# jrobine/actor-critic

Measured on AMD Instinct MI355X. Metric: env-steps/sec (whole node) + ACKTR update ms, Breakout 84x84x4, higher is better.
Workload: dtype fp32

## Files before the change

actor-critic_amd/actorcritic/_lib.py:

```python

import ctypes
import os

import torch

_HERE = os.path.dirname(os.path.abspath(__file__))
LIB_PATH = os.path.join(os.path.dirname(_HERE), 'libacmi.so')
if os.environ.get('ACMI_LIB'):
    LIB_PATH = os.environ['ACMI_LIB']

c_int = ctypes.c_int
c_i64 = ctypes.c_int64
c_u32 = ctypes.c_uint32
c_float = ctypes.c_float
c_vp = ctypes.c_void_p


class AcmiError(RuntimeError):
    """A libacmi entry point returned a non-zero status."""


class Net(ctypes.Structure):
    _fields_ = [('num_actions', c_int), ('conv3_filters', c_int), ('params', c_vp), ('conv_prep', c_vp),
                ('gemm_mode', c_int), ('forward_mode', c_int), ('conv_stats_mode', c_int)]


class Acts(ctypes.Structure):
    _fields_ = [('a1', c_vp), ('a2', c_vp), ('a3', c_vp), ('a4', c_vp),
                ('logits', c_vp), ('value', c_vp), ('ld_logits', c_int),
                ('ws', c_vp), ('ws_floats', c_i64), ('m1', c_vp), ('m2', c_vp), ('m3', c_vp)]


class Bwd(ctypes.Structure):
    _fields_ = [('d1', c_vp), ('d2', c_vp), ('d3', c_vp), ('d4', c_vp),
                ('dhead', c_vp), ('ldh', c_int)]


class EnvState(ctypes.Structure):
    _fields_ = [('episode', c_vp), ('step', c_vp), ('length', c_vp), ('total', c_vp), ('done', c_vp),
                ('game', c_vp)]


class RolloutIO(ctypes.Structure):
    _fields_ = [('seed', c_u32), ('stream_id', c_u32), ('counter', c_u32), ('counter_dev', c_vp),
                ('row_offset', c_int), ('actions', c_vp), ('bad_rows', c_vp), ('state', EnvState),
                ('env_offset', c_int), ('env_seed', c_u32), ('obs_out', c_vp), ('out_stride', c_i64),
                ('rewards', c_vp), ('terminals', c_vp), ('episode_rewards', c_vp), ('ld', c_i64),
                ('tower_done', c_int), ('next_acts', c_vp), ('next_act_stride', c_i64), ('obs_copy', c_vp)]


_SIGS = {
    'acmi_last_error': (ctypes.c_char_p, []),
    'acmi_abi_version': (c_int, []),
    'acmi_abi_struct_sizes': (c_int, [c_vp, c_int]),
    'acmi_set_forward_mode': (c_int, [c_int]),
    'acmi_get_forward_mode': (c_int, []),
    'acmi_set_gemm_mode': (c_int, [c_int]),
    'acmi_get_gemm_mode': (c_int, []),
    'acmi_set_conv_stats_mode': (c_int, [c_int]),
    'acmi_get_conv_stats_mode': (c_int, []),
    'acmi_band_info': (c_int, [c_int, c_int, c_i64, ctypes.POINTER(c_i64)]),
    'acmi_param_count': (c_i64, [c_int, c_int]),
    'acmi_conv_prep_bytes': (c_i64, [c_int]),
    'acmi_kfac_packed_floats': (c_i64, [c_int, c_int, c_int]),
    'acmi_kfac_pack': (c_int, [c_int, c_int, c_int, c_vp, c_vp, c_vp]),
    'acmi_kfac_unpack': (c_int, [c_int, c_int, c_int, c_vp, c_vp, c_vp]),
    'acmi_conv_prepare': (c_int, [ctypes.POINTER(Net), c_vp, c_vp]),
    'acmi_param_offsets': (c_int, [c_int, c_int, ctypes.POINTER(c_i64)]),
    'acmi_kfac_layout': (c_int, [c_int, c_int, ctypes.POINTER(c_i64), ctypes.POINTER(c_i64),
                                 ctypes.POINTER(c_i64), ctypes.POINTER(c_i64)]),
    'acmi_forward': (c_int, [ctypes.POINTER(Net), c_vp, c_i64, c_int, ctypes.POINTER(Acts), c_int, c_vp]),
    'acmi_forward_ws_floats': (c_i64, [c_int]),
    'acmi_forward_strided': (c_int, [ctypes.POINTER(Net), c_vp, c_i64, c_int, ctypes.POINTER(Acts), c_int,
                                     c_i64, c_vp]),
    'acmi_sample_actions': (c_int, [c_vp, c_int, c_int, c_int, c_u32, c_u32, c_u32, c_vp, c_int, c_vp,
                                    c_vp, c_vp]),
    'acmi_sample_actions_at': (c_int, [c_vp, c_int, c_int, c_int, c_u32, c_u32, c_u32, c_int, c_vp, c_int,
                                       c_vp, c_vp, c_vp]),
    'acmi_sample_actions_dev': (c_int, [c_vp, c_int, c_int, c_int, c_u32, c_u32, c_vp, c_u32, c_int, c_vp,
                                        c_int, c_vp, c_vp, c_vp]),
    'acmi_rollout_step': (c_int, [ctypes.POINTER(Net), c_vp, c_i64, c_int, ctypes.POINTER(Acts), c_i64,
                                  ctypes.POINTER(RolloutIO), c_vp]),
    'acmi_categorical': (c_int, [c_vp, c_int, c_int, c_int, c_vp, c_vp, c_vp, c_vp]),
    'acmi_returns': (c_int, [c_vp, c_vp, c_vp, c_vp, c_int, c_int, c_vp, c_vp, c_vp, c_vp, c_vp]),
    'acmi_gae': (c_int, [c_vp, c_vp, c_vp, c_vp, c_int, c_int, c_float, c_float, c_vp, c_vp, c_vp]),
    'acmi_adv_moments_ws_doubles': (c_i64, [c_i64]),
    'acmi_adv_moments': (c_int, [c_vp, c_i64, c_vp, c_vp, c_vp]),
    'acmi_adv_normalize': (c_int, [c_vp, c_i64, c_vp, ctypes.c_double, ctypes.c_double, c_vp]),
    'acmi_a2c_loss_ws_floats': (c_i64, [c_int]),
    'acmi_a2c_loss': (c_int, [c_vp, c_int, c_vp, c_vp, c_vp, c_vp, c_int, c_int, c_float, c_float, c_float,
                              c_vp, c_int, c_vp, c_vp, c_vp]),
    'acmi_ppo_loss_ws_floats': (c_i64, [c_int]),
    'acmi_ppo_loss': (c_int, [c_vp, c_int, c_vp, c_vp, c_vp, c_vp, c_vp, c_vp, c_int, c_int, c_float, c_float,
                              c_float, c_float, c_float, c_vp, c_int, c_vp, c_vp, c_vp, c_vp]),
    'acmi_backward_ws_floats': (c_i64, [c_int, c_int, c_int]),
    'acmi_backward': (c_int, [ctypes.POINTER(Net), c_vp, c_i64, c_int, ctypes.POINTER(Acts),
                              ctypes.POINTER(Bwd), c_vp, c_vp, c_vp, c_i64, c_vp]),
    'acmi_kfac_output_stats': (c_int, [ctypes.POINTER(Net), c_int, ctypes.POINTER(Acts), ctypes.POINTER(Bwd),
                                       c_u32, c_u32, c_u32, c_vp, c_vp, c_i64, c_vp]),
    'acmi_backward_stacked': (c_int, [ctypes.POINTER(Net), c_vp, c_i64, c_int, ctypes.POINTER(Acts),
                                      ctypes.POINTER(Bwd), c_vp, c_vp, c_vp, c_i64, ctypes.POINTER(Bwd), c_u32, c_u32,
                                      c_u32, c_vp, c_i64, c_vp]),
    'acmi_kfac_output_stats_finish': (c_int, [ctypes.POINTER(Net), c_int, ctypes.POINTER(Acts), ctypes.POINTER(Bwd),
                                              c_vp, c_vp, c_i64, c_vp]),
    'acmi_debug_ws_flushes': (c_int, []),
    'acmi_debug_convt2': (c_int, [ctypes.POINTER(Net), c_int, c_vp, c_vp, c_vp, c_vp, c_int, c_vp, c_vp, c_vp, c_vp,
                                  c_vp]),
    'acmi_kfac_ema': (c_int, [c_vp, c_vp, c_vp, c_i64, c_float, c_float, c_float, c_vp]),
    'acmi_kfac_inverse_layout': (c_int, [c_int, c_int, ctypes.POINTER(c_i64), ctypes.POINTER(c_i64)]),
    'acmi_kfac_inverse_floats': (c_i64, [c_int, c_int]),
    'acmi_kfac_inverse_ws_doubles': (c_i64, [c_int, c_int]),
    'acmi_kfac_inverse': (c_int, [c_int, c_int, c_vp, c_float, c_int, c_vp, c_vp, c_vp]),
    'acmi_kfac_eig_ws_doubles': (c_i64, [c_int, c_int]),
    'acmi_kfac_eigvals': (c_int, [c_int, c_int, c_vp, c_vp, c_vp, c_vp]),
    'acmi_kfac_step_ws_floats': (c_i64, [c_int, c_int]),
    'acmi_kfac_step': (c_int, [c_int, c_int, c_vp, c_vp, c_vp, c_vp, c_float, c_float, c_float, c_vp, c_vp,
                               c_vp, c_vp]),
    'acmi_opt_ws_floats': (c_i64, [c_i64]),
    'acmi_momentum_apply': (c_int, [c_vp, c_vp, c_vp, c_i64, c_float, c_float, c_float, c_vp, c_vp, c_vp]),
    'acmi_rmsprop_apply': (c_int, [c_vp, c_vp, c_vp, c_vp, c_i64, c_float, c_float, c_float, c_float, c_float,
                                   c_vp, c_vp, c_vp]),
    'acmi_adam_apply': (c_int, [c_vp, c_vp, c_vp, c_vp, c_i64, c_float, c_float, c_float, c_float, c_float,
                                c_vp, c_vp, c_vp]),
    'acmi_env_reset': (c_int, [ctypes.POINTER(EnvState), c_int, c_int, c_u32, c_vp, c_i64, c_vp]),
    'acmi_env_step': (c_int, [ctypes.POINTER(EnvState), c_int, c_int, c_u32, c_vp, c_vp, c_i64, c_vp, c_i64,
                              c_vp, c_vp, c_vp, c_i64, c_vp]),
    'acmi_atari_preprocess': (c_int, [c_vp, c_i64, c_i64, c_vp, c_int, c_int, c_int, c_vp, c_i64, c_vp]),
    'acmi_atari_stack': (c_int, [c_vp, c_i64, c_i64, c_vp, c_int, c_int, c_int, c_vp, c_int, c_vp, c_vp,
                                 c_i64, c_vp]),
    'acmi_stream_wait_backward_dx': (c_int, [c_vp]),
    'acmi_selftest_plans': (c_int, [c_int]),
    'acmi_gemm_f32': (c_int, [c_vp, c_vp, c_vp, c_int, c_int, c_int, c_vp]),
    'acmi_prof_enable': (c_int, [c_int, c_int]),
    'acmi_prof_collect': (c_int, [ctypes.POINTER(ctypes.c_double), ctypes.POINTER(c_int)]),
}

GEMM_F32 = 0
GEMM_X3 = 1
FWD_F32 = 0
FWD_BF16 = 1

CONV_STATS_PATCHES = 0
CONV_STATS_BAND = 1

PROF_CONV1_WGRAD = 1
PROF_CONV2_WGRAD = 2
PROF_CONV1_FWD = 3
PROF_CONV1_AFACTOR = 4
PROF_CONV2_DX = 5

EXPORTED = tuple(_SIGS)

_lib = None


def load():
    global _lib
    if _lib is None:
        if not os.path.exists(LIB_PATH):
            raise ImportError('libacmi.so not found at {} - build it with `python __graft_entry__.py build` '
                              '(hipcc --offload-arch=gfx950); there is no CPU fallback'.format(LIB_PATH))
        lib = ctypes.CDLL(LIB_PATH)
        for name, (res, args) in _SIGS.items():
            if os.environ.get('ACMI_LIB') and not hasattr(lib, name):
                continue
            fn = getattr(lib, name)
            fn.restype = res
            fn.argtypes = args
        if lib.acmi_abi_version() != 4:
            raise ImportError('libacmi ABI mismatch')
        _lib = lib
    return _lib


def check(status, what=''):
    if status != 0:
        msg = load().acmi_last_error().decode(errors='replace')
        raise AcmiError('{} failed ({}): {}'.format(what, status, msg))


def call(name, *args):
    check(getattr(load(), name)(*args), name)


def ptr(t):
    if t is None:
        return None
    assert t.is_contiguous(), 'libacmi needs contiguous buffers'
    return ctypes.c_void_p(t.data_ptr())

# ... 10 lines not shown
```

actor-critic_amd/csrc/convt2.hpp:

```cpp
#pragma once

#include "f16x2.hpp"
#include "gemm.hpp"

namespace acmi {

struct CT2 {
  static constexpr int CIN = 32, COUT = 64, OH = 9, OW = 9, PW = 10, L = 100;
  static constexpr int NKS = 16;
  static constexpr int STEP_BYTES = 4 * 2 * 1024;
  static constexpr int FRAG_BYTES = NKS * STEP_BYTES;
  static constexpr int BYTES = FRAG_BYTES + 4 * kAmaxWords;
  static constexpr int TILE = 128;
};

__device__ __forceinline__ void convt2_wmax_body(const float* w2, char* out, int b, int nb) {
  float m = 0.f;
  for (int i = b * 256 + threadIdx.x; i < 16 * CT2::CIN * CT2::COUT; i += nb * 256)
    m = fmaxf(m, fabsf(w2[i]));
  m = wave_max(m);
  if ((threadIdx.x & 63) == 0) amax_update(reinterpret_cast<unsigned*>(out + CT2::FRAG_BYTES), m);
}

__device__ __forceinline__ void convt2_prep_body(const float* w2, char* out, int blk) {
// ... 176 lines not shown
#pragma unroll
        for (int q = 0; q < 4; ++q) {
          float4 o;
          if constexpr (MASK) {
            o.x = (bits[q] & 1u) ? v[q].x : 0.f;
            o.y = (bits[q] & 2u) ? v[q].y : 0.f;
            o.z = (bits[q] & 4u) ? v[q].z : 0.f;
            o.w = (bits[q] & 8u) ? v[q].w : 0.f;
          } else {
            o.x = xa[q].x > 0.f ? v[q].x : 0.f;
            o.y = xa[q].y > 0.f ? v[q].y : 0.f;
            o.z = xa[q].z > 0.f ? v[q].z : 0.f;
            o.w = xa[q].w > 0.f ? v[q].w : 0.f;
          }
          if (jok[q]) {
            *reinterpret_cast<float4*>(d1 + (long long)(pix[q] + dp) * CT2::CIN + ri) = o;
            d1am = absmax4(d1am, o);
          }
        }
        __builtin_amdgcn_fence(__ATOMIC_RELEASE, "wavefront");
        __builtin_amdgcn_wave_barrier();
        __builtin_amdgcn_fence(__ATOMIC_ACQUIRE, "wavefront");
      }
    } else {
#pragma unroll
      for (int p = 0; p < 4; ++p) {
        const int py = p >> 1, px = p & 1;
        const long long pix = ((long long)n * 20 + 2 * Y + py) * 20 + 2 * X + px;
#pragma unroll
        for (int g = 0; g < 4; ++g) {
          const int ci = 8 * g + 4 * hl;
          float4 x;
          if constexpr (MASK) {
            const uint32_t b = *reinterpret_cast<const uint32_t*>(jok ? a1 + pix : zero) >> ci;
            x = make_float4((float)(b & 1u), (float)((b >> 1) & 1u), (float)((b >> 2) & 1u), (float)((b >> 3) & 1u));
          } else {
            x = *reinterpret_cast<const float4*>(jok ? a1 + pix * CT2::CIN + ci : zero);
          }
          const int c = lane & 31;
          scr[(ci + 0) * 36 + c] = x.x > 0.f ? acc[p][4 * g + 0] : 0.f;
          scr[(ci + 1) * 36 + c] = x.y > 0.f ? acc[p][4 * g + 1] : 0.f;
          scr[(ci + 2) * 36 + c] = x.z > 0.f ? acc[p][4 * g + 2] : 0.f;
          scr[(ci + 3) * 36 + c] = x.w > 0.f ? acc[p][4 * g + 3] : 0.f;
        }
        __builtin_amdgcn_wave_barrier();
#pragma unroll
        for (int h = 0; h < 2; ++h) {
          const float* rp = scr + (lane & 31) * 36 + 16 * h + 8 * hl;
          const float4 x0 = *reinterpret_cast<const float4*>(rp);
          const float4 x1 = *reinterpret_cast<const float4*>(rp + 4);
          uint4 hh, mm, ll;
          split3(x0.x, x0.y, hh.x, mm.x, ll.x);
          split3(x0.z, x0.w, hh.y, mm.y, ll.y);
          split3(x1.x, x1.y, hh.z, mm.z, ll.z);
          split3(x1.z, x1.w, hh.w, mm.w, ll.w);
          const bf16x8 f[3] = {__builtin_bit_cast(bf16x8, hh), __builtin_bit_cast(bf16x8, mm),
                               __builtin_bit_cast(bf16x8, ll)};
          gacc = mfma_x3(f, f, gacc);
        }
        __builtin_amdgcn_wave_barrier();
      }
    }
    __syncthreads();
  }

  if constexpr (MIX || !GRAM) amax_publish(d1max, d1am, lane);
  if constexpr (MIX || GRAM) {
    float* red = reinterpret_cast<float*>(lds);
    for (int w = 0; w < 4; ++w) {
      if (wave == w) {
#pragma unroll
        for (int r = 0; r < 16; ++r) {
          const int i = (r & 3) + 8 * (r >> 2) + 4 * hl, jc = lane & 31;
          red[i * 32 + jc] = (w ? red[i * 32 + jc] : 0.f) + gacc[r];
        }
      }
      __syncthreads();
    }
    float* out = gpart + (long long)blockIdx.x * 33 * 32;
    for (int e = tid; e < 32 * 32; e += 256) out[e] = red[e];
  }
}

#ifndef ACMI_CT2_STORE_BLOCKS
#define ACMI_CT2_STORE_BLOCKS 0
#endif
inline int convt2_store_blocks(int B) {
  const int ntiles = (B * CT2::L + CT2::TILE - 1) / CT2::TILE;
  return ACMI_CT2_STORE_BLOCKS > 0 ? std::max(1, std::min(ntiles, ACMI_CT2_STORE_BLOCKS)) : ntiles;
}
inline int convt2_gram_blocks(int B) {
  const int ntiles = (B * CT2::L + CT2::TILE - 1) / CT2::TILE;
  return std::max(1, std::min(ntiles, 768));
}

}
```

actor-critic_amd/csrc/net.hip:

```cpp
#include <math.h>
#include <stdlib.h>
#include <stdarg.h>
#include <stdio.h>
#include <string.h>

#include <vector>

#include "gemm.hpp"
#include "gemm3.hpp"
#include "conv1u8.hpp"
#include "convt3.hpp"
#include "convfwd3.hpp"
#include "band.hpp"
#include "tower.hpp"
#include "fc4roll.hpp"
#include "convt2.hpp"
#include "stepper.hpp"
#include "towersplit.hpp"

namespace acmi {

static int s_gemm_mode = [] {
  const char* e = getenv("ACMI_GEMM");
  return (e && e[0] == 'f') ? ACMI_GEMM_F32 : ACMI_GEMM_X3;
}();
static int s_conv_stats_mode = [] {
  const char* e = getenv("ACMI_BAND");
  return (e && e[0] == '0') ? ACMI_CONV_STATS_PATCHES : ACMI_CONV_STATS_BAND;
}();
static int s_forward_mode = [] {
  const char* e = getenv("ACMI_FORWARD");
  return (e && e[0] == 'b') ? ACMI_FWD_BF16 : ACMI_FWD_F32;
}();
thread_local int g_gemm_mode = s_gemm_mode;
thread_local int g_conv_stats_mode = s_conv_stats_mode;
thread_local int g_forward_mode = s_forward_mode;

static bool net_modes_ok(const acmi_net_t* n) {
  if (!n) return true;
  const int g = n->gemm_mode ? n->gemm_mode - 1 : s_gemm_mode;
  const int f = n->forward_mode ? n->forward_mode - 1 : s_forward_mode;
  const int c = n->conv_stats_mode ? n->conv_stats_mode - 1 : s_conv_stats_mode;
  return (g == ACMI_GEMM_F32 || g == ACMI_GEMM_X3) && (f == ACMI_FWD_F32 || f == ACMI_FWD_BF16) &&
         (c == ACMI_CONV_STATS_PATCHES || c == ACMI_CONV_STATS_BAND) && (f == ACMI_FWD_F32 || g == ACMI_GEMM_X3);
}
struct ModeScope {
  int g, f, c;
  explicit ModeScope(const acmi_net_t* n) : g(g_gemm_mode), f(g_forward_mode), c(g_conv_stats_mode) {
    g_gemm_mode = n && n->gemm_mode ? n->gemm_mode - 1 : s_gemm_mode;
    g_forward_mode = n && n->forward_mode ? n->forward_mode - 1 : s_forward_mode;
    g_conv_stats_mode = n && n->conv_stats_mode ? n->conv_stats_mode - 1 : s_conv_stats_mode;
  }
  ~ModeScope() {
    g_gemm_mode = g;
    g_forward_mode = f;
    g_conv_stats_mode = c;
  }
};

static thread_local char g_err[512];
void set_error(const char* fmt, ...) {
  va_list ap;
  va_start(ap, fmt);
  vsnprintf(g_err, sizeof(g_err), fmt, ap);
  va_end(ap);
}

static int g_prof_site = 0;
static int g_prof_cap = 0;
static int g_prof_n = 0;
static hipEvent_t* g_prof_ev = nullptr;

static void prof_begin(int site, hipStream_t s) {
  if (site != g_prof_site || g_prof_n >= g_prof_cap) return;
  (void)hipEventRecord(g_prof_ev[2 * g_prof_n], s);
}
static void prof_end(int site, hipStream_t s) {
  if (site != g_prof_site || g_prof_n >= g_prof_cap) return;
  (void)hipEventRecord(g_prof_ev[2 * g_prof_n + 1], s);
  ++g_prof_n;
}

struct Layout {
  int A, C3;
  long long off[12];
  long long total;
  long long K[6], N[6];
  long long din[6], dout[6];
// ... 1114 lines not shown
    }
    m = std::max(m, gcov_plan(co[l], rowsL[l]).floats);
  }
  m = std::max(m, band_ws_floats(band_host_plan(20, 20, 32, 4, 4, 2, 64), B));
  m = std::max(m, band_ws_floats(band_host_plan(9, 9, 64, 3, 3, 1, C3), B));
  return (m + 63) / 64 * 64;
}

static long long afactor_ws_floats(int B) { return conv1_afactor_ws_ints(400LL * B); }

static long long head_grad_ldg(int A) { return roundup4(A + 1) < 8 ? 8 : roundup4(A + 1); }
static long long bwd_prefix_floats(int B) { return kBandScratch + (afactor_ws_floats(B) + 63) / 64 * 64; }
static long long stats_prefix_floats(int B, int A) { return kBandScratch + ((long long)B * head_grad_ldg(A) + 63) / 64 * 64; }
static int g_ws_flushes = 0;

static hipEvent_t* dx_done_event() {
  static hipEvent_t ev[64] = {};
  int dev = 0;
  if (hipGetDevice(&dev) != hipSuccess || dev < 0 || dev >= 64) return nullptr;
  if (!ev[dev] && hipEventCreateWithFlags(&ev[dev], hipEventDisableTiming) != hipSuccess) {
    ev[dev] = nullptr;
    return nullptr;
  }
  return &ev[dev];
}
template <int C3>
static int dx_chain_pre(const Layout& L, const float* P, int B, const acmi_acts_t* a,
                        const acmi_bwd_t* bw, const float* dhead, int ldh,
                        hipStream_t s, const char* prep, unsigned* dxs) {
  ACMI_REQUIRE(dxs, ACMI_ERR_ARG, "dx_chain: no scratch");
  ACMI_REQUIRE(hipMemsetAsync(dxs, 0, kBandScratch * sizeof(unsigned), s) == hipSuccess, ACMI_ERR_HIP,
               "dx_chain: scratch reset failed");
  if (L.A == 4 && ldh % 4 == 0 && (uintptr_t)(P + L.off[8]) % 16 == 0 && (uintptr_t)dhead % 16 == 0)
    hipLaunchKernelGGL(heads_dx4_kernel, dim3(cdiv((long long)B * 128, 256)), dim3(256), 0, s, dhead,
                       ldh, B, P + L.off[8], P + L.off[10], a->a4, bw->d4, dxs + kBsMaxD4);
  else
    hipLaunchKernelGGL(heads_dx_kernel, dim3(cdiv((long long)B * 128, 256)), dim3(256), 0, s, dhead,
                       ldh, B, P + L.off[8], P + L.off[10], L.A, a->a4, bw->d4, dxs + kBsMaxD4);
  const unsigned* hdr = prep ? reinterpret_cast<const unsigned*>(prep + TowerPrep<C3>::HDR) : nullptr;
  const unsigned* w3max = hdr ? hdr + kTowMaxW3 : dxs + kBsMaxW3;
  const unsigned* w4max = hdr ? hdr + kTowMaxW4 : dxs + kBsMaxW4;
  if (!hdr && g_gemm_mode == ACMI_GEMM_X3) {
    hipLaunchKernelGGL(absmax_kernel, dim3(16), dim3(256), 0, s, P + L.off[4], (long long)576 * C3,
                       dxs + kBsMaxW3);
    hipLaunchKernelGGL(absmax_kernel, dim3(64), dim3(256), 0, s, P + L.off[6], (long long)49 * C3 * 512,
                       dxs + kBsMaxW4);
  }
  {
    const int K3 = 49 * C3;
    RowsAsK<DenseRows> opA{DenseRows{bw->d4, 512, B, 512}};
    MatTK<true> opB{P + L.off[6], 512, 512, K3};
    auto run = [&](auto epi) {
      if (g_gemm_mode == ACMI_GEMM_X3)
        launch_gemm3_f16<128, 64, 32, 2, 1>(opA, opB, epi, B, K3, 512, dxs + kBsMaxD4, w4max, s);
      else
        launch_mm<64, 128, 32, 1, 2, false, false, 16>(opA, opB, epi, B, K3, 512, 1, 0, s);
    };
    prof_begin(ACMI_PROF_FC4_DX, s);
    if (a->m3) run(EpiReluGrad<true>{bw->d3, reinterpret_cast<const float*>(a->m3), K3, dxs + kBsMaxD3});
    else run(EpiReluGrad<false>{bw->d3, a->a3, K3, dxs + kBsMaxD3});
    prof_end(ACMI_PROF_FC4_DX, s);
  }
  {
    const char* ct3p = prep ? prep + TowerPrep<C3>::BYTES + CT2::BYTES + fc4_prep_bytes(49 * C3) : nullptr;
    using Src = ConvTRows<9, 9, 3, 3, 1, C3>;
    using W = ConvTWeights<3, 3, 1, 64, C3>;
    W opA{P + L.off[4]};
    RowsAsK<Src> opB{Src{bw->d3, B * Src::L}};
    auto run = [&](auto epi) {
      if (g_gemm_mode == ACMI_GEMM_X3)
        launch_convt_x3<9, 9, 3, 3, 1, 64, C3, 256>(P + L.off[4], ct3p, bw->d3, B, epi, w3max, dxs + kBsMaxD3, s);
      else
        launch_mm<64, 128, 16, 1, 2, false, false, 16>(opA, opB, epi, W::N, B * Src::L, Src::COLS, 1, 0, s);
    };
    prof_begin(ACMI_PROF_CONV3_DX, s);
    if (a->m2) run(EpiConvT<9, 9, 1, 64, true>{bw->d2, reinterpret_cast<const float*>(a->m2), dxs + kBsMaxD2});
    else run(EpiConvT<9, 9, 1, 64>{bw->d2, a->a2, dxs + kBsMaxD2});
    prof_end(ACMI_PROF_CONV3_DX, s);
  }
  ACMI_LAUNCH_CHECK("dx_chain");
  return ACMI_OK;
}

template <int C3>
static int dx_conv2(const Layout& L, const float* P, int B, const acmi_acts_t* a, const acmi_bwd_t* bw,
                    hipStream_t s, const char* prep, float* gram_part, bool* gram_done, unsigned* dxs) {
  if (gram_done) *gram_done = false;
  {
    using Src = ConvTRows<20, 20, 4, 4, 2, 64>;
    using W = ConvTWeights<4, 4, 2, 32, 64>;
    W opA{P + L.off[2]};
    RowsAsK<Src> opB{Src{bw->d2, B * Src::L}};
    const float* act1 = a->m1 ? reinterpret_cast<const float*>(a->m1) : a->a1;
    prof_begin(ACMI_PROF_CONV2_DX, s);
    const char* p2 = prep ? prep + TowerPrep<C3>::BYTES : nullptr;
    if (p2 && g_gemm_mode == ACMI_GEMM_X3) {
      auto go = [&](auto GRAMc, auto MASKc) {
        constexpr bool GR = decltype(GRAMc)::value, MK = decltype(MASKc)::value;
        if (GR)
          hipLaunchKernelGGL((convt2_kernel<GR, MK>), dim3(convt2_gram_blocks(B)), dim3(256), 0, s, p2, bw->d2,
                             act1, nullptr, B, gram_part, dxs + kBsMaxD2, nullptr);
        else
          hipLaunchKernelGGL((convt2_kernel<GR, MK>), dim3(convt2_store_blocks(B)), dim3(256), 0, s, p2,
                             bw->d2, act1, bw->d1, B, nullptr, dxs + kBsMaxD2, dxs + kBsMaxD1);
      };
      using T = std::true_type;
      using F = std::false_type;
      if (gram_part) {
        if (a->m1) go(T{}, T{});
        else go(T{}, F{});
        if (gram_done) *gram_done = true;
      } else {
        if (a->m1) go(F{}, T{});
        else go(F{}, F{});
      }
    } else if (a->m1) {
      launch_mm<128, 128, 16, 2, 2, false, false, 16>(
          opA, opB, EpiConvT<20, 20, 2, 32, true>{bw->d1, act1, dxs + kBsMaxD1}, W::N, B * Src::L, Src::COLS, 1, 0, s);
    } else {
      launch_mm<128, 128, 16, 2, 2, false, false, 16>(opA, opB, EpiConvT<20, 20, 2, 32>{bw->d1, act1, dxs + kBsMaxD1},
                                                      W::N, B * Src::L, Src::COLS, 1, 0, s);
    }
    prof_end(ACMI_PROF_CONV2_DX, s);
  }
  ACMI_LAUNCH_CHECK("dx_conv2");
  return ACMI_OK;
}

template <int C3>
static int dx_chain(const Layout& L, const float* P, int B, const acmi_acts_t* a,
                    const acmi_bwd_t* bw, const float* dhead, int ldh,
                    hipStream_t s, const char* prep = nullptr, float* gram_part = nullptr,
                    bool* gram_done = nullptr, unsigned* dxs = nullptr) {
  const int rc = dx_chain_pre<C3>(L, P, B, a, bw, dhead, ldh, s, prep, dxs);
  if (rc) return rc;
  return dx_conv2<C3>(L, P, B, a, bw, s, prep, gram_part, gram_done, dxs);
}

template <int C3>
static int backward_impl(const Layout& L, const float* P, const uint8_t* obs,
                         long long img_stride, int B, const acmi_acts_t* a,
                         const acmi_bwd_t* bw, float* grads, float* astat,
                         float* ws, long long ws_cap, hipStream_t s, const char* prep,
                         bool dx_done = false) {
  const bool st = astat != nullptr;
  const bool fuse_c1 = st && g_gemm_mode == ACMI_GEMM_X3;
  unsigned* bscr = reinterpret_cast<unsigned*>(ws);
  const long long prefix = bwd_prefix_floats(B);
  float* part = ws + prefix;
  const long long avail = ws_cap - prefix;
  const bool band = band_on(st);
  int rc = ACMI_OK;
  if (!dx_done) {
    rc = dx_chain<C3>(L, P, B, a, bw, bw->dhead, bw->ldh, s, prep, nullptr, nullptr, bscr);
    if (rc) return rc;
    hipEvent_t* ev = dx_done_event();
    ACMI_REQUIRE(ev && hipEventRecord(*ev, s) == hipSuccess, ACMI_ERR_HIP, "acmi_backward: dX event record failed");
  }
  float* wpart_c1 = nullptr;
  if (st) {
    prof_begin(ACMI_PROF_CONV1_AFACTOR, s);
    const int rc0 = conv1_afactor_u8(obs, img_stride, B, astat + L.stat_off[0],
                                     reinterpret_cast<int*>(ws + kBandScratch), afactor_ws_floats(B), s,
                                     fuse_c1 ? bw->d1 : nullptr, &wpart_c1, bscr + kBsMaxD1);
    prof_end(ACMI_PROF_CONV1_AFACTOR, s);
    if (rc0) return rc0;
  }
  WgradSet fin;
  long long off = 0;
  auto flush = [&]() {
    if (fin.n) hipLaunchKernelGGL(finalize_wgrad_multi_kernel, dim3(fin.blocks), dim3(256), 0, s, fin);
    fin = WgradSet();
    off = 0;
  };
  if (st && fuse_c1) {
    const long long rows = 400LL * B;
    WgradDesc d{wpart_c1, conv1_afactor_fused_chunks(rows), 256, 32, 0, 32, grads + L.off[0], 32,
                nullptr, nullptr, (int)rows, 1.0f / 255.0f};
    fin.add(d, 0, 0, fin_blocks(d));
  }
  auto layer = [&](long long need, auto&& run) -> int {
    long long used = 0;
// ... 509 lines not shown
  const char* prep = static_cast<const char*>(net->conv_prep);
  if (L.C3 == 32)
    return output_stats_impl<32>(L, net->params, B, acts, bwd_s, 0, 0, 0, g_stats, ws_s, ws_s_floats, s, prep, 2);
  return output_stats_impl<64>(L, net->params, B, acts, bwd_s, 0, 0, 0, g_stats, ws_s, ws_s_floats, s, prep, 2);
}

int acmi_stream_wait_backward_dx(acmi_stream_t stream) {
  hipEvent_t* ev = dx_done_event();
  ACMI_REQUIRE(ev && hipStreamWaitEvent((hipStream_t)stream, *ev, 0) == hipSuccess, ACMI_ERR_HIP,
               "acmi_stream_wait_backward_dx failed");
  return ACMI_OK;
}

int acmi_kfac_output_stats(const acmi_net_t* net, int B, const acmi_acts_t* acts,
                           const acmi_bwd_t* bwd, uint32_t seed, uint32_t row_offset,
                           uint32_t counter, float* g_stats, float* ws, int64_t ws_floats,
                           acmi_stream_t stream) {
  ACMI_REQUIRE(net_modes_ok(net), ACMI_ERR_ARG, "acmi_kfac_output_stats: bad acmi_net_t mode fields");
  const ModeScope mode_scope(net);
  Layout L;
  ACMI_REQUIRE(net && acts && bwd && g_stats && ws, ACMI_ERR_ARG,
               "acmi_kfac_output_stats: null argument");
  ACMI_REQUIRE(make_layout(net->num_actions, net->conv3_filters, &L), ACMI_ERR_ARG, "bad net");
  ACMI_REQUIRE(B > 0 && spans32(B, 400 * 32, 400 * 32), ACMI_ERR_ARG, "bad B");
  ACMI_REQUIRE(masks_ok(acts), ACMI_ERR_ARG, "acmi_kfac_output_stats: ReLU masks m1..m3 must be all set or all NULL");
  const long long need = acmi_backward_ws_floats(B, net->num_actions, net->conv3_filters);
  ACMI_REQUIRE(ws_floats >= need, ACMI_ERR_WS, "acmi_kfac_output_stats: workspace of %lld floats < %lld",
               (long long)ws_floats, need);
  hipStream_t s = (hipStream_t)stream;
  if (L.C3 == 32)
    return output_stats_impl<32>(L, net->params, B, acts, bwd, seed, row_offset, counter,
                                 g_stats, ws, ws_floats, s, static_cast<const char*>(net->conv_prep));
  return output_stats_impl<64>(L, net->params, B, acts, bwd, seed, row_offset, counter, g_stats,
                               ws, ws_floats, s, static_cast<const char*>(net->conv_prep));
}

int acmi_prof_enable(int site, int capacity) {
  ACMI_REQUIRE(site >= 0 && capacity >= 0 && capacity <= 65536, ACMI_ERR_ARG,
               "acmi_prof_enable: bad site/capacity");
  if (g_prof_ev) {
    for (int i = 0; i < 2 * g_prof_cap; ++i) (void)hipEventDestroy(g_prof_ev[i]);
    delete[] g_prof_ev;
    g_prof_ev = nullptr;
  }
  g_prof_site = 0;
  g_prof_cap = 0;
  g_prof_n = 0;
  if (site == 0 || capacity == 0) return ACMI_OK;
  g_prof_ev = new hipEvent_t[2 * capacity];
  for (int i = 0; i < 2 * capacity; ++i) {
    if (hipEventCreate(&g_prof_ev[i]) != hipSuccess) {
      set_error("acmi_prof_enable: hipEventCreate failed");
      return ACMI_ERR_HIP;
    }
  }
  g_prof_site = site;
  g_prof_cap = capacity;
  return ACMI_OK;
}

int acmi_prof_collect(double* total_ms, int* count) {
  ACMI_REQUIRE(total_ms && count, ACMI_ERR_ARG, "acmi_prof_collect: null argument");
  double t = 0.0;
  for (int i = 0; i < g_prof_n; ++i) {
    if (hipEventSynchronize(g_prof_ev[2 * i + 1]) != hipSuccess) {
      set_error("acmi_prof_collect: hipEventSynchronize failed");
      return ACMI_ERR_HIP;
    }
    float ms = 0.f;
    (void)hipEventElapsedTime(&ms, g_prof_ev[2 * i], g_prof_ev[2 * i + 1]);
    t += ms;
  }
  *total_ms = t;
  *count = g_prof_n;
  g_prof_n = 0;
  return ACMI_OK;
}

int acmi_debug_convt2(const acmi_net_t* net, int mode, const float* d2a, const float* d2b, const uint32_t* m1,
                      float* d1, int B, float* gram_part, const uint32_t* d2max_a, const uint32_t* d2max_b,
                      uint32_t* d1max, acmi_stream_t stream) {
  ACMI_REQUIRE(net_modes_ok(net), ACMI_ERR_ARG, "acmi_debug_convt2: bad acmi_net_t mode fields");
  const ModeScope mode_scope(net);
  ACMI_REQUIRE(net && net->conv_prep && d2a && d2b && m1 && d1 && gram_part && d2max_a && d2max_b && d1max && B > 0,
               ACMI_ERR_ARG, "acmi_debug_convt2: bad arguments");
  const char* p2 = static_cast<const char*>(net->conv_prep) +
                   (net->conv3_filters == 32 ? TowerPrep<32>::BYTES : TowerPrep<64>::BYTES);
  hipStream_t s = (hipStream_t)stream;
  const float* act1 = reinterpret_cast<const float*>(m1);
  if (mode == 0) {
    hipLaunchKernelGGL((convt2_kernel<false, true>), dim3(convt2_store_blocks(B)), dim3(256), 0, s, p2, d2a, act1, d1,
                       B, nullptr, d2max_a, d1max, nullptr, nullptr);
    hipLaunchKernelGGL((convt2_kernel<true, true>), dim3(convt2_gram_blocks(B)), dim3(256), 0, s, p2, d2b, act1,
                       nullptr, B, gram_part, d2max_b, nullptr, nullptr, nullptr);
  } else {
    hipLaunchKernelGGL((convt2_kernel<true, true, true>), dim3(convt2_gram_blocks(B)), dim3(256), 0, s, p2, d2a,
                       act1, d1, B, gram_part, d2max_a, d1max, d2b, d2max_b);
  }
  ACMI_LAUNCH_CHECK("acmi_debug_convt2");
  return ACMI_OK;
}

int acmi_debug_ws_flushes(void) {
  const int n = g_ws_flushes;
  g_ws_flushes = 0;
  return n;
}

int acmi_selftest_plans(int max_k) {
  for (int K = 64; K <= max_k; K += 32) {
    SymPlan p;
    if (!sym_plan(K, 64, &p)) continue;
    const int J = K + 64;
    std::vector<unsigned char> cov((size_t)K * J, 0);
    std::vector<int> cs(J, 0);
    for (int g = 0; g < p.ngroups; ++g)
      for (int w = 0; w < 4; ++w) {
        if (p.g[g].wa[w] < 0) continue;
        const int a = p.g[g].base[p.g[g].wa[w]], b = p.g[g].base[p.g[g].wb[w]];
        if (a < 0 || b < 0 || a >= K) return K;
        for (int i = a; i < a + 64 && i < K; ++i)
          for (int j = b; j < b + 64 && j < J; ++j) cov[(size_t)i * J + j] = 1;
        if (a == 0)
          for (int j = b; j < b + 64 && j < J; ++j) cs[j]++;
      }
    for (int i = 0; i < K; ++i)
      for (int j = i; j < J; ++j)
        if (!cov[(size_t)i * J + j]) return K;
    for (int j = 0; j < J; ++j)
      if (cs[j] < 1) return K;
  }
  for (int K : {512, 576})
    for (int cp : {8, 32, 64}) {
      SymPlan6 p;
      if (!sym_plan6(K, cp, &p)) return -(K + cp);
      const int nb = K / 64;
      std::vector<int> cov((size_t)(nb + 1) * (nb + 1), 0), cs(nb + 1, 0);
      for (int g = 0; g < p.ngroups; ++g) {
        int n = 0;
        for (int w = 0; w < 8; ++w)
          for (int t = 0; t < 2; ++t) {
            const int ra = p.g[g].ra[w][t], cb = p.g[g].cb[w][t];
            if (ra < 0) {
              if (t == 0 && p.g[g].ra[w][1] >= 0) return -(K + cp);
              continue;
            }
            ++n;
            const int a = p.g[g].base[ra], b = p.g[g].base[cb];
            if (a < 0 || b < 0 || a % 64 || a >= K || b < a) return -(K + cp);
            cov[(size_t)(a / 64) * (nb + 1) + b / 64]++;
            if (a == 0) cs[b / 64]++;
            if (t == 1 && p.g[g].base[p.g[g].cb[w][0]] == K && b != K) return -(K + cp);
          }
        if (n > 16) return -(K + cp);
      }
      for (int a = 0; a < nb; ++a)
        for (int b = a; b <= nb; ++b)
          if (cov[(size_t)a * (nb + 1) + b] != 1) return -(K + cp);
      for (int b = 0; b <= nb; ++b)
        if (cs[b] != 1) return -(K + cp);
    }
  for (int K : {1568, 512, 576})
    for (int cp : {512, 64, 8}) {
      SymPlan6 p;
      if (!sym_plan6_greedy(K, cp, &p)) return -(K + cp + 1);
      const int J = K + cp, ns = (J + 63) / 64, nbp = (K + 63) / 64;
      std::vector<int> cov((size_t)ns * ns, 0), cs(ns, 0);
      for (int g = 0; g < p.ngroups; ++g) {
        int n = 0;
        for (int w = 0; w < 8; ++w) {
          bool half0 = false;
          for (int t = 0; t < 2; ++t) {
            const int ra = p.g[g].ra[w][t], cb = p.g[g].cb[w][t];
            if (ra < 0) {
              if (t == 0 && p.g[g].ra[w][1] >= 0) return -(K + cp + 1);
              continue;
            }
            ++n;
            const int a = p.g[g].base[ra], b = p.g[g].base[cb];
            const bool half = b + 32 >= J;
            if (t == 0) half0 = half;
            else if (half0 && !half) return -(K + cp + 1);
            if (a % 64 || b % 64 || a >= K || b < a || b >= J) return -(K + cp + 1);
// ... 48 lines not shown
```

include/acmi.h:

```cpp
#ifndef ACMI_H_
#define ACMI_H_

#include <stdint.h>

#ifdef __cplusplus
extern "C" {
#endif

#define ACMI_ABI_VERSION 4

enum {
  ACMI_OK = 0,
  ACMI_ERR_ARG = -1,
  ACMI_ERR_HIP = -2,
  ACMI_ERR_WS = -3,
};

typedef void* acmi_stream_t;

const char* acmi_last_error(void);
int acmi_abi_version(void);
int acmi_abi_struct_sizes(int64_t* sizes, int n);

#define ACMI_GEMM_F32 0
// ... 163 lines not shown
int64_t acmi_kfac_step_ws_floats(int num_actions, int conv3_filters);
int acmi_kfac_step(int num_actions, int conv3_filters, float* params,
                   float* velocity, const float* grads, const float* inv,
                   float lr, float momentum, float norm_constraint,
                   float* precon, float* ws, float* coeff_out,
                   acmi_stream_t stream);

int64_t acmi_opt_ws_floats(int64_t n);
int acmi_momentum_apply(float* params, float* accum, const float* grads,
                        int64_t n, float lr, float momentum, float clip_norm,
                        float* ws, float* norm_out, acmi_stream_t stream);
int acmi_rmsprop_apply(float* params, float* ms, float* mom,
                       const float* grads, int64_t n, float lr, float decay,
                       float momentum, float eps, float clip_norm, float* ws,
                       float* norm_out, acmi_stream_t stream);
int acmi_adam_apply(float* params, float* m, float* v, const float* grads,
                    int64_t n, float lr_t, float beta1, float beta2, float eps,
                    float clip_norm, float* ws, float* norm_out,
                    acmi_stream_t stream);

typedef struct acmi_env_state {
  int32_t* episode;
  int32_t* step;
  int32_t* length;
  float* total;
  uint8_t* done;
  const uint8_t* game;
} acmi_env_state_t;

int acmi_env_reset(const acmi_env_state_t* st, int N, int env_offset,
                   uint32_t seed, uint8_t* obs_out, int64_t out_stride,
                   acmi_stream_t stream);
int acmi_env_step(const acmi_env_state_t* st, int N, int env_offset,
                  uint32_t seed, const int32_t* actions, const uint8_t* obs_in,
                  int64_t in_stride, uint8_t* obs_out, int64_t out_stride,
                  float* rewards, uint8_t* terminals, float* episode_rewards,
                  int64_t ld, acmi_stream_t stream);

int acmi_atari_preprocess(const uint8_t* raw, int64_t env_stride,
                          int64_t frame_stride, const uint8_t* nframes, int N,
                          int H, int W, uint8_t* gray_out, int64_t out_stride,
                          acmi_stream_t stream);
int acmi_atari_stack(const uint8_t* raw, int64_t env_stride, int64_t frame_stride,
                     const uint8_t* nframes, int N, int H, int W,
                     const uint8_t* terminals, int reset, const uint8_t* stack_in,
                     uint8_t* stack_out, int64_t stack_stride, acmi_stream_t stream);

int acmi_forward_strided(const acmi_net_t* net, const uint8_t* obs,
                         int64_t img_stride, int B, const acmi_acts_t* acts,
                         int want_value, int64_t act_img_stride,
                         acmi_stream_t stream);

typedef struct acmi_rollout_io {
  uint32_t seed, stream_id, counter;
  const uint32_t* counter_dev;
  int row_offset;
  int32_t* actions;
  int32_t* bad_rows;
  acmi_env_state_t state;
  int env_offset;
  uint32_t env_seed;
  uint8_t* obs_out;
  int64_t out_stride;
  float* rewards;
  uint8_t* terminals;
  float* episode_rewards;
  int64_t ld;
  int tower_done;
  const struct acmi_acts* next_acts;
  int64_t next_act_stride;
  uint8_t* obs_copy;
} acmi_rollout_io_t;
int acmi_rollout_step(const acmi_net_t* net, const uint8_t* obs,
                      int64_t img_stride, int B, const acmi_acts_t* acts,
                      int64_t act_img_stride, const acmi_rollout_io_t* io,
                      acmi_stream_t stream);

int acmi_selftest_plans(int max_k);
int acmi_debug_ws_flushes(void);
int acmi_debug_convt2(const acmi_net_t* net, int mode, const float* d2a, const float* d2b,
                      const uint32_t* m1, float* d1, int B, float* gram_part,
                      const uint32_t* d2max_a, const uint32_t* d2max_b, uint32_t* d1max,
                      acmi_stream_t stream);

int acmi_gemm_f32(const float* A, const float* B, float* C, int M, int N,
                  int K, acmi_stream_t stream);

#define ACMI_PROF_CONV1_WGRAD 1
#define ACMI_PROF_CONV2_WGRAD 2
#define ACMI_PROF_CONV1_FWD 3
#define ACMI_PROF_CONV1_AFACTOR 4
#define ACMI_PROF_CONV2_DX 5
#define ACMI_PROF_FC4_DX 6
#define ACMI_PROF_CONV3_DX 7
int acmi_prof_enable(int site, int capacity);
int acmi_prof_collect(double* total_ms, int* count);

#ifdef __cplusplus
}
#endif
#endif
```

Measured before the change: 2.911 million.

## Add LDS-resident weight conv2 transpose kernel with persistent multi-team blocks

Adds a conv2 input-gradient kernel variant that loads the full W2^T f16 fragment set into LDS once per block. Each block runs three 256-thread teams that loop persistently over tiles, prefetching the next tile's d2 taps while the MFMAs run. This removes the repeated global weight fragment reads of the per-tile kernel, at the cost of very large LDS use (one block per CU) and more complex scheduling. It is enabled by default only for very large batches (at least 2000 tiles), with a debug switch to force either form.

```diff
diff --git a/actor-critic_amd/actorcritic/_lib.py b/actor-critic_amd/actorcritic/_lib.py
--- a/actor-critic_amd/actorcritic/_lib.py
+++ b/actor-critic_amd/actorcritic/_lib.py
@@ -106,6 +106,7 @@
     'acmi_debug_ws_flushes': (c_int, []),
     'acmi_debug_convt2': (c_int, [ctypes.POINTER(Net), c_int, c_vp, c_vp, c_vp, c_vp, c_int, c_vp, c_vp, c_vp, c_vp,
                                   c_vp]),
+    'acmi_debug_convt2_form': (c_int, [c_int]),
     'acmi_kfac_ema': (c_int, [c_vp, c_vp, c_vp, c_i64, c_float, c_float, c_float, c_vp]),
     'acmi_kfac_inverse_layout': (c_int, [c_int, c_int, ctypes.POINTER(c_i64), ctypes.POINTER(c_i64)]),
     'acmi_kfac_inverse_floats': (c_i64, [c_int, c_int]),
diff --git a/actor-critic_amd/csrc/convt2.hpp b/actor-critic_amd/csrc/convt2.hpp
--- a/actor-critic_amd/csrc/convt2.hpp
+++ b/actor-critic_amd/csrc/convt2.hpp
@@ -282,6 +282,296 @@
   }
 }
 
+struct CT2R {
+  static constexpr int TEAMS = 3, THREADS = TEAMS * 256, WAVES = THREADS / 64;
+  static constexpr int STORE_LD = 36, GRAM_LD = 20;
+  static constexpr int WAVE_SCR = 4 * std::max(16 * STORE_LD, 32 * GRAM_LD);
+  static constexpr int LDS_BYTES = CT2::FRAG_BYTES + WAVES * WAVE_SCR;
+  static constexpr int MAX_TEAMS = 768;
+};
+static_assert(CT2R::LDS_BYTES <= 163840, "resident W2^T fragments + epilogue scratch exceed a CU's 160 KiB of LDS");
+static_assert(4 * CT2R::WAVE_SCR >= 32 * 32 * 4, "a team's Gram sum red[32][32] aliases its four waves' scratch");
+static_assert(CT2R::WAVE_SCR % 16 == 0 && CT2::FRAG_BYTES % (16 * 64) == 0, "16-byte LDS rows");
+
+__device__ __attribute__((weak, aligned(16))) float kCt2ZeroPixel[CT2::COUT] = {};
+
+template <bool GRAM, bool MASK>
+__global__ __launch_bounds__(CT2R::THREADS)
+void convt2_resident_kernel(const char* prep, const float* __restrict__ d2, const float* __restrict__ a1,
+                            float* __restrict__ d1, int B, float* __restrict__ gpart, const unsigned* d2max,
+                            unsigned* d1max, int G) {
+  __shared__ __attribute__((aligned(16))) char lds[CT2R::LDS_BYTES];
+  const int tid = threadIdx.x, lane = tid & 63;
+  const int bwave = __builtin_amdgcn_readfirstlane(tid >> 6);
+  const int wave = bwave & 3, team = bwave >> 2;
+  const int J = B * CT2::L;
+  const int ntiles = (J + CT2::TILE - 1) / CT2::TILE;
+  const int v = CT2R::TEAMS * blockIdx.x + team;
+  const bool active = v < G;
+  const int hl = lane >> 5;
+  const float* zero = zero_run();
+  const float sd = f16x2_scale_of_bits(d2max);
+  const float sw = f16x2_scale_of_bits(reinterpret_cast<const unsigned*>(prep + CT2::FRAG_BYTES));
+  const float inv = 1.f / (sw * sd);
+
+  float d1am = 0.f;
+  f32x16 gacc;
+#pragma unroll
+  for (int r = 0; r < 16; ++r) gacc[r] = 0.f;
+
+  struct Col {
+    bool ok;
+    int n, Y, X;
+    const float* dimg;
+  };
+  auto col_of = [&](int tile) {
+    Col c;
+    const int j = tile * CT2::TILE + 32 * wave + (lane & 31);
+    c.ok = j < J;
+    const int jj = c.ok ? j : 0;
+    c.n = jj / CT2::L;
+    const int sp = jj - c.n * CT2::L;
+    c.Y = sp / CT2::PW;
+    c.X = sp - c.Y * CT2::PW;
+    c.dimg = d2 + (long long)c.n * (CT2::OH * CT2::OW * CT2::COUT);
+    return c;
+  };
+  auto tap_ptr = [&](int t, bool cok, int Y, int X, const float* dimg) {
+    const int a = t >> 1, b = t & 1;
+    const int oy = Y - a, ox = X - b;
+    const bool ok = cok & (oy >= 0) & (oy < CT2::OH) & (ox >= 0) & (ox < CT2::OW);
+    const int oyc = max(oy, 0), oxc = max(ox, 0);
+    const float* p = dimg + (oyc * CT2::OW + oxc) * CT2::COUT;
+    return (ok ? p : kCt2ZeroPixel) + 8 * hl;
+  };
+  auto bload = [&](const float* p, int cg, float4 (&x)[2]) {
+    x[0] = *reinterpret_cast<const float4*>(p + 16 * cg);
+    x[1] = *reinterpret_cast<const float4*>(p + 16 * cg + 4);
+  };
+
+  float4 bx0[2], bx1[2], bx2[2], bx3[2];
+  Col cur = col_of(min(v, ntiles - 1));
+  const float* pc = tap_ptr(0, cur.ok, cur.Y, cur.X, cur.dimg);
+  bload(pc, 0, bx0);
+  bload(pc, 1, bx1);
+
+  {
+    constexpr int RUNS = CT2::FRAG_BYTES / 16, PER = (RUNS + CT2R::THREADS - 1) / CT2R::THREADS;
+    const uint4* src = reinterpret_cast<const uint4*>(prep);
+    uint4* dst = reinterpret_cast<uint4*>(lds);
+    uint4 r[PER];
+#pragma unroll
+    for (int k = 0; k < PER; ++k) r[k] = src[min(tid + CT2R::THREADS * k, RUNS - 1)];
+#pragma unroll
+    for (int k = 0; k < PER; ++k)
+      if (tid + CT2R::THREADS * k < RUNS) dst[tid + CT2R::THREADS * k] = r[k];
+  }
+  __syncthreads();
+
+  float* scr = reinterpret_cast<float*>(lds + CT2::FRAG_BYTES + bwave * CT2R::WAVE_SCR);
+  const bool amax_per_tile = (G & (kAmaxSlots - 1)) != 0;
+  auto publish_d1max = [&](int tile) {
+    const float m = wave_max(d1am);
+    if (d1max && lane == 0) {
+      unsigned* q = d1max + kAmaxStride * (tile & (kAmaxSlots - 1));
+      const unsigned u = __float_as_uint(m);
+      if (u > __hip_atomic_load(q, __ATOMIC_RELAXED, __HIP_MEMORY_SCOPE_AGENT)) atomicMax(q, u);
+    }
+  };
+
+  for (int tile = active ? v : ntiles; tile < ntiles; tile += G) {
+    const Col nextc = col_of(min(tile + G, ntiles - 1));
+    const bool jok = cur.ok;
+    const int n = cur.n, Y = cur.Y, X = cur.X;
+
+    f32x16 acc[4];
+#pragma unroll
+    for (int p = 0; p < 4; ++p)
+#pragma unroll
+      for (int r = 0; r < 16; ++r) acc[p][r] = 0.f;
+
+    auto step = [&](const char* As, const float4 (&cb)[2], auto&& loads) {
+      loads();
+      __builtin_amdgcn_sched_barrier(0);
+      auto aread = [&](int p, f16x8 (&a)[2]) {
+#pragma unroll
+        for (int q = 0; q < 2; ++q) a[q] = as_f16x8(*reinterpret_cast<const uint4*>(As + (p * 2 + q) * 1024));
+      };
+      f16x8 b[2], a0[2], a1[2];
+      aread(0, a0);
+      split2x8(cb[0], cb[1], sd, b[0], b[1]);
+      aread(1, a1);
+      acc[0] = mfma_x2(a0, b, acc[0]);
+      aread(2, a0);
+      acc[1] = mfma_x2(a1, b, acc[1]);
+      aread(3, a1);
+      acc[2] = mfma_x2(a0, b, acc[2]);
+      acc[3] = mfma_x2(a1, b, acc[3]);
+      __builtin_amdgcn_sched_group_barrier(0x100, 2, 0);
+      __builtin_amdgcn_sched_group_barrier(0x002, 64, 0);
+      __builtin_amdgcn_sched_group_barrier(0x100, 2, 0);
+      __builtin_amdgcn_sched_group_barrier(0x008, 3, 0);
+      __builtin_amdgcn_sched_group_barrier(0x100, 2, 0);
+      __builtin_amdgcn_sched_group_barrier(0x008, 3, 0);
+      __builtin_amdgcn_sched_group_barrier(0x100, 2, 0);
+      __builtin_amdgcn_sched_group_barrier(0x008, 6, 0);
+      __builtin_amdgcn_sched_barrier(0);
+    };
+#pragma unroll 1
+    for (int t = 0; t < 4; ++t) {
+      const bool wrap = t == 3;
+      const float* pn = tap_ptr((t + 1) & 3, wrap ? nextc.ok : cur.ok, wrap ? nextc.Y : cur.Y,
+                                wrap ? nextc.X : cur.X, wrap ? nextc.dimg : cur.dimg);
+      const char* As = lds + t * (4 * CT2::STEP_BYTES) + lane * 16;
+      step(As, bx0, [&] { bload(pc, 2, bx2); bload(pc, 3, bx3); });
+      step(As + CT2::STEP_BYTES, bx1, [] {});
+      step(As + 2 * CT2::STEP_BYTES, bx2, [&] { bload(pn, 0, bx0); bload(pn, 1, bx1); });
+      step(As + 3 * CT2::STEP_BYTES, bx3, [] {});
+      pc = pn;
+    }
+    cur = nextc;
+#pragma unroll
+    for (int p = 0; p < 4; ++p)
+#pragma unroll
+      for (int r = 0; r < 16; ++r) acc[p][r] *= inv;
+
+    const int half = (lane >> 4) & 1;
+    if constexpr (!GRAM) {
+      const int ri = 4 * (lane & 7), cj = lane >> 3;
+      int pix[4];
+      bool qok[4];
+#pragma unroll
+      for (int q = 0; q < 4; ++q) {
+        const int j = tile * CT2::TILE + 32 * wave + cj + 8 * q;
+        qok[q] = j < J;
+        const int jj = qok[q] ? j : 0;
+        const int nn = jj / CT2::L, sp = jj - nn * CT2::L;
+        const int yy = sp / CT2::PW, xx = sp - yy * CT2::PW;
+        pix[q] = (nn * 20 + 2 * yy) * 20 + 2 * xx;
+      }
+#pragma unroll
+      for (int p = 0; p < 4; ++p) {
+        const int dp = (p >> 1) * 20 + (p & 1);
+        uint32_t bits[4];
+        float4 xa[4];
+#pragma unroll
+        for (int q = 0; q < 4; ++q) {
+          const int px = pix[q] + dp;
+          if constexpr (MASK) bits[q] = reinterpret_cast<const uint32_t*>(qok[q] ? a1 + px : zero)[0] >> ri;
+          else xa[q] = *reinterpret_cast<const float4*>(qok[q] ? a1 + px * CT2::CIN + ri : zero);
+        }
+#pragma unroll
+        for (int h = 0; h < 2; ++h) {
+          if (half == h) {
+#pragma unroll
+            for (int g = 0; g < 4; ++g)
+              *reinterpret_cast<float4*>(scr + (lane & 15) * CT2R::STORE_LD + 8 * g + 4 * hl) =
+                  make_float4(acc[p][4 * g], acc[p][4 * g + 1], acc[p][4 * g + 2], acc[p][4 * g + 3]);
+          }
+          __builtin_amdgcn_fence(__ATOMIC_RELEASE, "wavefront");
+          __builtin_amdgcn_wave_barrier();
+          __builtin_amdgcn_fence(__ATOMIC_ACQUIRE, "wavefront");
+#pragma unroll
+          for (int q = 2 * h; q < 2 * h + 2; ++q) {
+            const float4 x = *reinterpret_cast<const float4*>(scr + (cj + 8 * (q - 2 * h)) * CT2R::STORE_LD + ri);
+            float4 o;
+            if constexpr (MASK) {
+              o.x = (bits[q] & 1u) ? x.x : 0.f;
+              o.y = (bits[q] & 2u) ? x.y : 0.f;
+              o.z = (bits[q] & 4u) ? x.z : 0.f;
+              o.w = (bits[q] & 8u) ? x.w : 0.f;
+            } else {
+              o.x = xa[q].x > 0.f ? x.x : 0.f;
+              o.y = xa[q].y > 0.f ? x.y : 0.f;
+              o.z = xa[q].z > 0.f ? x.z : 0.f;
+              o.w = xa[q].w > 0.f ? x.w : 0.f;
+            }
+            if (qok[q]) {
+              *reinterpret_cast<float4*>(d1 + (long long)(pix[q] + dp) * CT2::CIN + ri) = o;
+              d1am = absmax4(d1am, o);
+            }
+          }
+          __builtin_amdgcn_fence(__ATOMIC_RELEASE, "wavefront");
+          __builtin_amdgcn_wave_barrier();
+          __builtin_amdgcn_fence(__ATOMIC_ACQUIRE, "wavefront");
+        }
+      }
+      if (amax_per_tile) {
+        publish_d1max(tile);
+        d1am = 0.f;
+      }
+    } else {
+#pragma unroll
+      for (int p = 0; p < 4; ++p) {
+        const int py = p >> 1, px = p & 1;
+        const long long pix = ((long long)n * 20 + 2 * Y + py) * 20 + 2 * X + px;
+#pragma unroll
+        for (int g = 0; g < 4; ++g) {
+          const int ci = 8 * g + 4 * hl;
+          float4 x;
+          if constexpr (MASK) {
+            const uint32_t b = *reinterpret_cast<const uint32_t*>(jok ? a1 + pix : zero) >> ci;
+            x = make_float4((float)(b & 1u), (float)((b >> 1) & 1u), (float)((b >> 2) & 1u), (float)((b >> 3) & 1u));
+          } else {
+            x = *reinterpret_cast<const float4*>(jok ? a1 + pix * CT2::CIN + ci : zero);
+          }
+          acc[p][4 * g + 0] = x.x > 0.f ? acc[p][4 * g + 0] : 0.f;
+          acc[p][4 * g + 1] = x.y > 0.f ? acc[p][4 * g + 1] : 0.f;
+          acc[p][4 * g + 2] = x.z > 0.f ? acc[p][4 * g + 2] : 0.f;
+          acc[p][4 * g + 3] = x.w > 0.f ? acc[p][4 * g + 3] : 0.f;
+        }
+#pragma unroll
+        for (int h = 0; h < 2; ++h) {
+          if (half == h) {
+#pragma unroll
+            for (int r = 0; r < 16; ++r)
+              scr[((r & 3) + 8 * (r >> 2) + 4 * hl) * CT2R::GRAM_LD + (lane & 15)] = acc[p][r];
+          }
+          __builtin_amdgcn_fence(__ATOMIC_RELEASE, "wavefront");
+          __builtin_amdgcn_wave_barrier();
+          __builtin_amdgcn_fence(__ATOMIC_ACQUIRE, "wavefront");
+          const float* rp = scr + (lane & 31) * CT2R::GRAM_LD + 8 * hl;
+          const float4 x0 = *reinterpret_cast<const float4*>(rp);
+          const float4 x1 = *reinterpret_cast<const float4*>(rp + 4);
+          uint4 hh, mm, ll;
+          split3(x0.x, x0.y, hh.x, mm.x, ll.x);
+          split3(x0.z, x0.w, hh.y, mm.y, ll.y);
+          split3(x1.x, x1.y, hh.z, mm.z, ll.z);
+          split3(x1.z, x1.w, hh.w, mm.w, ll.w);
+          const bf16x8 f[3] = {__builtin_bit_cast(bf16x8, hh), __builtin_bit_cast(bf16x8, mm),
+                               __builtin_bit_cast(bf16x8, ll)};
+          gacc = mfma_x3(f, f, gacc);
+          __builtin_amdgcn_fence(__ATOMIC_RELEASE, "wavefront");
+          __builtin_amdgcn_wave_barrier();
+          __builtin_amdgcn_fence(__ATOMIC_ACQUIRE, "wavefront");
+        }
+      }
+    }
+  }
+
+  if constexpr (!GRAM) {
+    if (active) publish_d1max(v);
+  }
+  __syncthreads();
+  if constexpr (GRAM) {
+    float* red = reinterpret_cast<float*>(lds + CT2::FRAG_BYTES + team * 4 * CT2R::WAVE_SCR);
+    for (int w = 0; w < 4; ++w) {
+      if (wave == w) {
+#pragma unroll
+        for (int r = 0; r < 16; ++r) {
+          const int i = (r & 3) + 8 * (r >> 2) + 4 * hl, jc = lane & 31;
+          red[i * 32 + jc] = (w ? red[i * 32 + jc] : 0.f) + gacc[r];
+        }
+      }
+      __syncthreads();
+    }
+    if (active) {
+      float* out = gpart + (long long)v * 33 * 32;
+      for (int e = tid & 255; e < 32 * 32; e += 256) out[e] = red[e];
+    }
+  }
+}
+
 #ifndef ACMI_CT2_STORE_BLOCKS
 #define ACMI_CT2_STORE_BLOCKS 0
 #endif
@@ -293,5 +583,20 @@
   const int ntiles = (B * CT2::L + CT2::TILE - 1) / CT2::TILE;
   return std::max(1, std::min(ntiles, 768));
 }
-
-}
+inline int convt2_resident_teams(int B) { return convt2_gram_blocks(B); }
+inline int convt2_resident_blocks(int B) { return (convt2_resident_teams(B) + CT2R::TEAMS - 1) / CT2R::TEAMS; }
+static_assert(CT2R::MAX_TEAMS == 768 && CT2R::MAX_TEAMS % kAmaxSlots == 0, "teams = convt2_gram_blocks");
+#ifndef ACMI_CT2R_MIN_TILES_STORE
+#define ACMI_CT2R_MIN_TILES_STORE 2000
+#endif
+#ifndef ACMI_CT2R_MIN_TILES_GRAM
+#define ACMI_CT2R_MIN_TILES_GRAM 2000
+#endif
+constexpr int kCt2ResidentMinTilesStore = ACMI_CT2R_MIN_TILES_STORE;
+constexpr int kCt2ResidentMinTilesGram = ACMI_CT2R_MIN_TILES_GRAM;
+inline bool convt2_resident_default(int B, bool gram) {
+  const int ntiles = (B * CT2::L + CT2::TILE - 1) / CT2::TILE;
+  return ntiles >= (gram ? kCt2ResidentMinTilesGram : kCt2ResidentMinTilesStore);
+}
+
+}
diff --git a/actor-critic_amd/csrc/net.hip b/actor-critic_amd/csrc/net.hip
--- a/actor-critic_amd/csrc/net.hip
+++ b/actor-critic_amd/csrc/net.hip
@@ -4,6 +4,7 @@
 #include <stdio.h>
 #include <string.h>
 
+#include <atomic>
 #include <vector>
 
 #include "gemm.hpp"
@@ -1284,6 +1285,12 @@
   return ACMI_OK;
 }
 
+static std::atomic<int> g_convt2_form{-1};
+static bool convt2_use_resident(int B, bool gram) {
+  const int f = g_convt2_form.load(std::memory_order_relaxed);
+  return f < 0 ? convt2_resident_default(B, gram) : f != 0;
+}
+
 template <int C3>
 static int dx_conv2(const Layout& L, const float* P, int B, const acmi_acts_t* a, const acmi_bwd_t* bw,
                     hipStream_t s, const char* prep, float* gram_part, bool* gram_done, unsigned* dxs) {
@@ -1299,7 +1306,11 @@
     if (p2 && g_gemm_mode == ACMI_GEMM_X3) {
       auto go = [&](auto GRAMc, auto MASKc) {
         constexpr bool GR = decltype(GRAMc)::value, MK = decltype(MASKc)::value;
-        if (GR)
+        if (convt2_use_resident(B, GR))
+          hipLaunchKernelGGL((convt2_resident_kernel<GR, MK>), dim3(convt2_resident_blocks(B)), dim3(CT2R::THREADS),
+                             0, s, p2, bw->d2, act1, GR ? nullptr : bw->d1, B, GR ? gram_part : nullptr,
+                             dxs + kBsMaxD2, GR ? nullptr : dxs + kBsMaxD1, convt2_resident_teams(B));
+        else if (GR)
           hipLaunchKernelGGL((convt2_kernel<GR, MK>), dim3(convt2_gram_blocks(B)), dim3(256), 0, s, p2, bw->d2,
                              act1, nullptr, B, gram_part, dxs + kBsMaxD2, nullptr);
         else
@@ -1975,7 +1986,8 @@
                       uint32_t* d1max, acmi_stream_t stream) {
   ACMI_REQUIRE(net_modes_ok(net), ACMI_ERR_ARG, "acmi_debug_convt2: bad acmi_net_t mode fields");
   const ModeScope mode_scope(net);
-  ACMI_REQUIRE(net && net->conv_prep && d2a && d2b && m1 && d1 && gram_part && d2max_a && d2max_b && d1max && B > 0,
+  ACMI_REQUIRE(net && net->conv_prep && d2a && d2b && m1 && d1 && gram_part && d2max_a && d2max_b && d1max && B > 0 &&
+                   mode >= 0 && mode <= 2,
                ACMI_ERR_ARG, "acmi_debug_convt2: bad arguments");
   const char* p2 = static_cast<const char*>(net->conv_prep) +
                    (net->conv3_filters == 32 ? TowerPrep<32>::BYTES : TowerPrep<64>::BYTES);
@@ -1986,12 +1998,22 @@
                        B, nullptr, d2max_a, d1max, nullptr, nullptr);
     hipLaunchKernelGGL((convt2_kernel<true, true>), dim3(convt2_gram_blocks(B)), dim3(256), 0, s, p2, d2b, act1,
                        nullptr, B, gram_part, d2max_b, nullptr, nullptr, nullptr);
-  } else {
+  } else if (mode == 1) {
     hipLaunchKernelGGL((convt2_kernel<true, true, true>), dim3(convt2_gram_blocks(B)), dim3(256), 0, s, p2, d2a,
                        act1, d1, B, gram_part, d2max_a, d1max, d2b, d2max_b);
+  } else {
+    const dim3 grid(convt2_resident_blocks(B)), block(CT2R::THREADS);
+    hipLaunchKernelGGL((convt2_resident_kernel<false, true>), grid, block, 0, s, p2, d2a, act1, d1, B, nullptr,
+                       d2max_a, d1max, convt2_resident_teams(B));
+    hipLaunchKernelGGL((convt2_resident_kernel<true, true>), grid, block, 0, s, p2, d2b, act1, nullptr, B, gram_part,
+                       d2max_b, nullptr, convt2_resident_teams(B));
   }
   ACMI_LAUNCH_CHECK("acmi_debug_convt2");
   return ACMI_OK;
+}
+
+int acmi_debug_convt2_form(int form) {
+  return g_convt2_form.exchange(form < 0 ? -1 : form != 0, std::memory_order_relaxed);
 }
 
 int acmi_debug_ws_flushes(void) {
diff --git a/include/acmi.h b/include/acmi.h
--- a/include/acmi.h
+++ b/include/acmi.h
@@ -269,6 +269,7 @@
                       const uint32_t* m1, float* d1, int B, float* gram_part,
                       const uint32_t* d2max_a, const uint32_t* d2max_b, uint32_t* d1max,
                       acmi_stream_t stream);
+int acmi_debug_convt2_form(int form);
 
 int acmi_gemm_f32(const float* A, const float* B, float* C, int M, int N,
                   int K, acmi_stream_t stream);
```

New measurement: 2.964 million (median of 6 runs). 1.8% higher.
